# GMichailov/Flash-Attention-CUDA-C

Measured on AMD Instinct MI355X. Metric: fwd attention TFLOP/s/GPU (bf16, seq=4096, d=128) + % MFMA peak, higher is better.
Workload: dtype bf16

## Files before the change

flash-attention-cuda-c_amd/csrc/computers.hip.h:

```cpp
#pragma once

#include "slot_engine.hip.h"

namespace fa {

template <int R>
struct Scores {
    f32x16 s[R][2];
};

template <class C>
struct WaveCompute : SlotEngine<WaveCompute<C>, C> {
    static constexpr int D = C::D, ESZ = C::ESZ, R = 1;
    static constexpr int KS = D / 16;
    static constexpr int DB = D / 32;
    static constexpr int NA = 2 * KS, NB = 4 * DB;
    static constexpr int SA = NA * R, SB = NB * R;
    static constexpr int MPF = ESZ == 1 ? 2 : 1;
    static constexpr int NF = NA / MPF;
    static constexpr int FPH = NF / 2;
    static constexpr int NPRE = C::NPRE < NF ? C::NPRE : NF;
    static constexpr int VPRE = C::VPRE;
    static constexpr int GROUPS = R, RG = 32, LOG_RG = 5, FPG = FPH;
    static constexpr int NE = 32 * R;
    static constexpr int SPAN = SA + (3 * SB) / 4;
    using G = TileGeom<D, ESZ>;
    using Stage = std::conditional_t<C::MIX, MixStage<D, C::NWAVES>,
                  std::conditional_t<C::DMA, DmaStage<D, C::NWAVES, false, true>,
                                     std::conditional_t<C::DMA_K8, HybridStageFp8<D, C::NWAVES>, BufStage<D, ESZ, C::NWAVES, C::PAD>>>>;
    using ScoresT = Scores<R>;
    static constexpr int NL = Stage::NL, NW = Stage::NW;

    u32x4 qf[R][FPH];
    f32x16 o[R][DB];
    float m[R];
    float l[R];
    u32x4 kf[NPRE];
    bf16x8 vf[VPRE + 1];
    uint32_t pw[R][16];
    float sum_a[R], sum_b[R], mx_a[R], mx_b[R], p_even, p_last;
    bool need;
    unsigned long long t_mid = 0, t_end = 0;

    __device__ __forceinline__ void init() {
#pragma unroll
        for (int r = 0; r < R; ++r) {
#pragma unroll
            for (int i = 0; i < DB; ++i)
#pragma unroll
                for (int k = 0; k < 16; ++k) o[r][i][k] = 0.f;
            m[r] = -INFINITY;
            l[r] = 0.f;
        }
    }

    __host__ __device__ static constexpr int frag_u(int f) { return f % FPH; }
    __host__ __device__ static constexpr int frag_kt(int f) { return f / FPH; }
    __device__ __forceinline__ u32x4 k_read(lds_ptr kimg, int kbase, int f) const {
        if constexpr (Stage::K_DMA) return __builtin_bit_cast(u32x4, lds_read_b128(kimg, kbase + frag_kt(f) * (4 * Stage::KBLK) + frag_u(f) * 256));
        else return __builtin_bit_cast(u32x4, lds_read_b128(kimg, kbase + frag_u(f) * 2048 + frag_kt(f) * 512));
    }
    template <int F, int SUB, int RG>
    __device__ __forceinline__ void qk_mfma(const u32x4& kprev, const u32x4& kfrag, Scores<R>& n) const {
        const u32x4& q = qf[RG][frag_u(F)];
        f32x16& acc = n.s[RG][frag_kt(F)];
        if constexpr (C::MXQK) {
            static_assert(ESZ == 1, "the MX form is for fp8 inputs");
            if constexpr ((F & 1) && SUB == MPF - 1) acc = mfma_32x32x64_fp8_unit_scale(kprev, kfrag, qf[RG][(F - 1) % FPH], q, acc);
        } else {
            static_assert(ESZ == 2, "the non-scaled form is for bf16 inputs");
            acc = mfma_32x32x16(__builtin_bit_cast(bf16x8, kfrag), __builtin_bit_cast(bf16x8, q), acc);
        }
    }
    __device__ __forceinline__ static void zero(Scores<R>& n) {
#pragma unroll
        for (int r = 0; r < R; ++r)
#pragma unroll
            for (int k = 0; k < 16; ++k) { n.s[r][0][k] = 0.f; n.s[r][1][k] = 0.f; }
    }

    template <int I = 0>
    __device__ __forceinline__ void qk_all(lds_ptr kimg, int kbase, Scores<R>& n) {
        if constexpr (I == 0) zero(n);
        if constexpr (I < SA) {
            constexpr int f = I / (MPF * R), sub = (I % (MPF * R)) / R, rg = I % R;
            if constexpr (I % (MPF * R) == 0) kf[f % 2] = k_read(kimg, kbase, f);
            qk_mfma<f, sub, rg>(kf[(f + 1) % 2], kf[f % 2], n);
            qk_all<I + 1>(kimg, kbase, n);
        }
    }

    __device__ __forceinline__ void mask(Scores<R>& n, int kv0, int q_row0, int S, int lane) const {
        const int k0 = kv0 + 4 * (lane >> 5);
#pragma unroll
        for (int r = 0; r < R; ++r) {
            const int qi = q_row0 + 32 * r + (lane & 31);
            const int lim = C::CAUSAL ? (qi < S - 1 ? qi : S - 1) : S - 1;
#pragma unroll
            for (int k = 0; k < 16; ++k) {
                n.s[r][0][k] = (k0 + acc_row(k, 0)) > lim ? -INFINITY : n.s[r][0][k];
                n.s[r][1][k] = (k0 + 32 + acc_row(k, 0)) > lim ? -INFINITY : n.s[r][1][k];
            }
        }
    }
    __device__ __forceinline__ float row_max(const Scores<R>& n, int r) const {
        float a = fmaxf(n.s[r][0][0], n.s[r][0][1]), b = fmaxf(n.s[r][1][0], n.s[r][1][1]);
#pragma unroll
        for (int k = 2; k < 16; k += 2) {
            a = fmaxf(a, fmaxf(n.s[r][0][k], n.s[r][0][k + 1]));
            b = fmaxf(b, fmaxf(n.s[r][1][k], n.s[r][1][k + 1]));
        }
        return fmaxf(a, b);
    }
    __device__ __forceinline__ static float max_over_row(float x) { return max_both_halves(x); }

    template <int E, bool F16W = false>
    __device__ __forceinline__ void exp_elem(const Scores<R>& cur, float c) {
        constexpr int g = E / (8 * R), r = (E / 8) % R, j = E % 8, e = 8 * g + j;
        const float x = cur.s[r][e >> 4][e & 15];
        if constexpr (C::LATE_ADD) {
            if constexpr (E > 0) {
                constexpr int rp = ((E - 1) / 8) % R, ep = 8 * ((E - 1) / (8 * R)) + (E - 1) % 8;
                if constexpr (ep & 1) sum_b[rp] += p_last;
                else sum_a[rp] += p_last;
                asm volatile("" : "+v"(sum_a[rp]), "+v"(sum_b[rp]));
            }
            const float p = fast_exp2(fmaf(x, c, -m[r]));
            p_last = p;
            if constexpr (e & 1) pw[r][e >> 1] = F16W ? pack_f16(p_even, p) : pack_bf16(p_even, p);
            else p_even = p;
        } else {
            const float p = fast_exp2(fmaf(x, c, -m[r]));
            if constexpr (e & 1) {
                sum_b[r] += p;
                pw[r][e >> 1] = F16W ? pack_f16(p_even, p) : pack_bf16(p_even, p);
                asm volatile("" : "+v"(sum_a[r]), "+v"(sum_b[r]));
            } else {
                sum_a[r] += p;
                p_even = p;
            }
        }
    }
    __device__ __forceinline__ bf16x8 p_frag(int r, int g) const {
        u32x4 v = {pw[r][4 * g], pw[r][4 * g + 1], pw[r][4 * g + 2], pw[r][4 * g + 3]};
        return __builtin_bit_cast(bf16x8, v);
    }
    template <int J>
    __device__ __forceinline__ void max3_slot(const Scores<R>& n) {
        constexpr int PER = 64 / NB;
#pragma unroll
        for (int k = 0; k < PER; k += 2) {
            const int E = J * PER + k, r = E / 32, e = E % 32;
            const float x0 = n.s[r][e >> 4][e & 15];
            const float x1 = n.s[r][(e + 1) >> 4][(e + 1) & 15];
            if ((k >> 1) & 1) mx_b[r] = fmaxf(fmaxf(mx_b[r], x0), x1);
            else mx_a[r] = fmaxf(fmaxf(mx_a[r], x0), x1);
        }
#pragma unroll
        for (int r = 0; r < R; ++r) asm volatile("" : "+v"(mx_a[r]), "+v"(mx_b[r]));
    }

    __device__ __forceinline__ bf16x8 v_frag(lds_ptr vimg, int vbase, int s4, int db) const {
        const s16x4 lo = lds_read_tr16_b64(vimg, vbase + (2 * s4) * (DB * 512) + db * 512);
        const s16x4 hi = lds_read_tr16_b64(vimg, vbase + (2 * s4 + 1) * (DB * 512) + db * 512);
        typedef __attribute__((ext_vector_type(8))) short s16x8;
        return __builtin_bit_cast(bf16x8, (s16x8)__builtin_shufflevector(lo, hi, 0, 1, 2, 3, 4, 5, 6, 7));
    }

    template <int I, bool F16W = false>
    __device__ __forceinline__ void slots_a(Stage& st, int t_load, lds_ptr k_next, lds_ptr v_cur, int kbase, int vbase,
                                            float c, const Scores<R>& cur, Scores<R>& nxt) {
        if constexpr (I < SA) {
            constexpr int f = I / (MPF * R), rem = I % (MPF * R), sub = rem / R, rg = rem % R;
            if constexpr (C::VALU_FIRST) this->template exp_slot<I, F16W>(cur, c);
            qk_mfma<f, sub, rg>(kf[(f + NPRE - 1) % NPRE], kf[f % NPRE], nxt);
            if constexpr (C::MXQK) {
                if constexpr (rem == MPF * R - 1 && (f & 1)) {
                    if constexpr (f - 1 + NPRE < NF) kf[(f - 1) % NPRE] = k_read(k_next, kbase, f - 1 + NPRE);
                    if constexpr (f + NPRE < NF) kf[f % NPRE] = k_read(k_next, kbase, f + NPRE);
                }
            } else if constexpr (rem == MPF * R - 1 && f + NPRE < NF) {
                kf[f % NPRE] = k_read(k_next, kbase, f + NPRE);
            }
            if constexpr (I >= SA - VPRE) {
                constexpr int v = I - (SA - VPRE);
                vf[v % (VPRE + 1)] = v_frag(v_cur, vbase, v / DB, v % DB);
            }
            this->template load_in_slot<I, F16W>(st, t_load);
            if constexpr (!C::VALU_FIRST) this->template exp_slot<I, F16W>(cur, c);
            __builtin_amdgcn_sched_barrier(0);
            slots_a<I + 1, F16W>(st, t_load, k_next, v_cur, kbase, vbase, c, cur, nxt);
        }
    }
    template <bool TRACK, int J, bool F16W = false>
    __device__ __forceinline__ void slots_b(Stage& st, lds_ptr wr_slot, lds_ptr v_cur, int vbase, float c,
                                            const Scores<R>& cur, const Scores<R>& nxt) {
        if constexpr (J < SB) {
            constexpr int v = J / R, rg = J % R, s4 = v / DB, db = v % DB;
            if constexpr (F16W) o[rg][db] = mfma_32x32x16(__builtin_bit_cast(f16x8, vf[v % (VPRE + 1)]), __builtin_bit_cast(f16x8, p_frag(rg, s4)), o[rg][db]);
            else o[rg][db] = mfma_32x32x16(vf[v % (VPRE + 1)], p_frag(rg, s4), o[rg][db]);
            if constexpr (rg == R - 1 && v + VPRE < NB) {
                constexpr int vn = v + VPRE;
                vf[vn % (VPRE + 1)] = v_frag(v_cur, vbase, vn / DB, vn % DB);
            }
            this->template exp_slot<SA + J, F16W>(cur, c);
            if constexpr (TRACK && J < SB / 2) max3_slot<J>(nxt);
            if constexpr (TRACK && J == SB / 2) this->decide(c);
            this->template write_in_slot<J, F16W>(st, wr_slot);
            __builtin_amdgcn_sched_barrier(0);
            slots_b<TRACK, J + 1, F16W>(st, wr_slot, v_cur, vbase, c, cur, nxt);
        }
    }

    __device__ __forceinline__ void begin_tile(Stage& st, lds_ptr wr_slot, Scores<R>& nxt) {
        st.set_dst(wr_slot);
#pragma unroll
        for (int r = 0; r < R; ++r) {
            sum_a[r] = sum_b[r] = 0.f;
            mx_a[r] = mx_b[r] = -INFINITY;
        }
        zero(nxt);
    }
    __device__ __forceinline__ void end_sums() {
        if constexpr (C::LATE_ADD) {
            static_assert(((NE - 1) % 8) & 1, "the last element feeds sum_b");
            sum_b[((NE - 1) / 8) % R] += p_last;
        }
#pragma unroll
        for (int r = 0; r < R; ++r) l[r] += sum_a[r] + sum_b[r];
    }
    __device__ __forceinline__ void rescale(int r, float alpha) {
        l[r] *= alpha;
#pragma unroll
        for (int i = 0; i < DB; ++i)
#pragma unroll
            for (int k = 0; k < 16; ++k) o[r][i][k] *= alpha;
    }

    __device__ __forceinline__ bool not_finite() const {
        float acc[4] = {0.f, 0.f, 0.f, 0.f};
#pragma unroll
        for (int r = 0; r < R; ++r) {
            acc[0] = fmaf(l[r], 0.f, acc[0]);
#pragma unroll
            for (int i = 0; i < DB; ++i)
#pragma unroll
                for (int k = 0; k < 16; ++k) acc[k & 3] = fmaf(o[r][i][k], 0.f, acc[k & 3]);
        }
        const float a = (acc[0] + acc[1]) + (acc[2] + acc[3]);
        return a != a;
    }

    template <typename OutT>
    __device__ __forceinline__ void store_o_lds(lds_ptr region, char* Oh, float* lse_head, int64_t oS_bytes, int row0, int S,
                                                int lane, int orow_bytes = D * 2) {
        static_assert(sizeof(OutT) == 2, "LDS epilogue is for bf16 / f16 outputs");
        constexpr int ROWB = D * 2, CHUNKS = ROWB / 16;
        const int q = lane & 31, h = lane >> 5;
#pragma unroll
        for (int r = 0; r < R; ++r) {
            const float l_tot = sum_both_halves(l[r]);
            this->store_lse(lse_head, l_tot, r, row0, S, lane);
            const float inv = 1.0f / l_tot;
#pragma unroll
            for (int db = 0; db < DB; ++db)
#pragma unroll
                for (int g4 = 0; g4 < 4; ++g4) {
                    const int d0 = 32 * db + 8 * g4 + 4 * h;
                    const float a = o[r][db][4 * g4 + 0] * inv, b = o[r][db][4 * g4 + 1] * inv;
                    const float c2 = o[r][db][4 * g4 + 2] * inv, e = o[r][db][4 * g4 + 3] * inv;
                    u32x2 v;
                    if constexpr (__is_same(OutT, __bf16)) v = u32x2{pack_bf16(a, b), pack_bf16(c2, e)};
                    else v = u32x2{pack_f16(a, b), pack_f16(c2, e)};
                    const int chunk = (d0 * 2) >> 4, half8 = (d0 * 2) & 8;
                    *reinterpret_cast<FA_LDS u32x2*>(region + (32 * r + q) * ROWB + (((chunk ^ q) & (CHUNKS - 1)) << 4) + half8) = v;
                }
        }
        __builtin_amdgcn_s_waitcnt(0xc07f);
        constexpr int ROWS_PER_INST = 64 / CHUNKS;
        const int rr = lane / CHUNKS, cc = lane % CHUNKS;
        if (!C::PAD && row0 + 32 * R <= S) {
            u32x4 v[32 * R / ROWS_PER_INST];
#pragma unroll
            for (int i = 0; i < 32 * R / ROWS_PER_INST; ++i) {
                const int row = i * ROWS_PER_INST + rr;
                v[i] = *reinterpret_cast<FA_LDS const u32x4*>(region + row * ROWB + (((cc ^ row) & (CHUNKS - 1)) << 4));
            }
#pragma unroll
            for (int i = 0; i < 32 * R / ROWS_PER_INST; ++i)
                store_global_b128<C::O_CACHE>(Oh + (int64_t)(row0 + i * ROWS_PER_INST + rr) * oS_bytes + cc * 16, v[i]);
            return;
        }
#pragma unroll
        for (int i = 0; i < 32 * R / ROWS_PER_INST; ++i) {
            const int row = i * ROWS_PER_INST + rr;
            const u32x4 v = *reinterpret_cast<FA_LDS const u32x4*>(region + row * ROWB + (((cc ^ row) & (CHUNKS - 1)) << 4));
            if (row0 + row < S && (!C::PAD || cc * 16 < orow_bytes))
                *reinterpret_cast<u32x4*>(Oh + (int64_t)(row0 + row) * oS_bytes + cc * 16) = v;
        }
    }
    template <typename OutT>
    __device__ __forceinline__ void store_o_lds32(lds_ptr region, char* Oh, float* lse_head, int64_t oS_bytes, int row0, int S,
                                                  int lane, int orow_bytes = D * 4) {
        static_assert(sizeof(OutT) == 4, "for fp32 outputs");
        const int q = lane & 31, h = lane >> 5;
        float inv[R];
#pragma unroll
        for (int r = 0; r < R; ++r) {
            const float l_tot = sum_both_halves(l[r]);
            this->store_lse(lse_head, l_tot, r, row0, S, lane);
            inv[r] = 1.0f / l_tot;
        }
        const int rr = lane >> 4, cc = lane & 15;
#pragma unroll
        for (int hf = 0; hf < D / 64; ++hf) {
            if (hf > 0) __builtin_amdgcn_s_waitcnt(0xc07f);
#pragma unroll
            for (int r = 0; r < R; ++r)
#pragma unroll
                for (int dd = 0; dd < 2; ++dd)
#pragma unroll
                    for (int g4 = 0; g4 < 4; ++g4) {
                        const int db = 2 * hf + dd, cidx = 8 * dd + 2 * g4 + h;
                        const f32x4 v = {o[r][db][4 * g4 + 0] * inv[r], o[r][db][4 * g4 + 1] * inv[r],
                                         o[r][db][4 * g4 + 2] * inv[r], o[r][db][4 * g4 + 3] * inv[r]};
                        *reinterpret_cast<FA_LDS f32x4*>(region + (32 * r + q) * 256 + (((cidx ^ q) & 15) << 4)) = v;
                    }
            __builtin_amdgcn_s_waitcnt(0xc07f);
            if (!C::PAD && row0 + 32 * R <= S) {
                f32x4 v[8 * R];
#pragma unroll
                for (int i = 0; i < 8 * R; ++i) v[i] = *reinterpret_cast<FA_LDS const f32x4*>(region + (4 * i + rr) * 256 + (((cc ^ (4 * i + rr)) & 15) << 4));
#pragma unroll
                for (int i = 0; i < 8 * R; ++i) store_global_b128<C::O_CACHE>(Oh + (int64_t)(row0 + 4 * i + rr) * oS_bytes + hf * 256 + cc * 16, __builtin_bit_cast(u32x4, v[i]));
                continue;
            }
#pragma unroll
            for (int i = 0; i < 8 * R; ++i) {
                const int row = 4 * i + rr;
                const f32x4 v = *reinterpret_cast<FA_LDS const f32x4*>(region + row * 256 + (((cc ^ row) & 15) << 4));
                if (row0 + row < S && (!C::PAD || hf * 256 + cc * 16 < orow_bytes))
                    *reinterpret_cast<f32x4*>(Oh + (int64_t)(row0 + row) * oS_bytes + hf * 256 + cc * 16) = v;
            }
        }
    }
};

}
```

flash-attention-cuda-c_amd/csrc/kernel_bf16.hip.h:

```cpp
#pragma once

#include "computers.hip.h"
#include "computers16.hip.h"

#include <type_traits>

namespace fa {

struct Opt {
    bool stamp = false;
    bool pad = false;
    int m16 = -1;
    int sum_mfma = -1;
    int waves = 8;
    bool p_f16 = false;
    bool mix = false;
    int kv_clamp = -1;
    int q_nt = -1;
};

template <int D_, bool CAUSAL_, typename OutT_, int ESZ_ = 2, Opt O = Opt{}>
struct KernelCfg {
    static constexpr int D = D_;
    static constexpr bool CAUSAL = CAUSAL_;
    using OutT = OutT_;
    static constexpr int ESZ = ESZ_;
    static constexpr bool STAMP = O.stamp, PAD = O.pad;
    static constexpr bool PRIO_A = true;
    static constexpr int O_CACHE = CAUSAL_ ? 2 : 0;
    static constexpr int Q_CACHE = (O.q_nt < 0 ? CAUSAL_ : O.q_nt != 0) ? 2 : 0;
    static constexpr bool KV_CLAMP = CAUSAL_ && O.kv_clamp != 0;
    static constexpr bool COALESCED_Q = D_ == 128 && !O.pad;
    static constexpr bool MXQK = ESZ_ == 1;
    static constexpr bool M16 = (O.m16 < 0 ? true : O.m16 != 0) && ESZ_ == 2;
    static constexpr bool SUM_MFMA = M16 && (O.sum_mfma < 0 ? true : O.sum_mfma != 0);
    static constexpr bool VALU_FIRST = !M16;
    static constexpr bool P_F16 = M16 && O.p_f16;
    static constexpr bool LATE_ADD = !M16;
    static constexpr bool DMA = ESZ_ == 2 && !O.pad && !O.p_f16;
    static constexpr bool MIX = O.mix && DMA;
    static_assert(!O.mix || (ESZ_ == 2 && !O.pad && !O.p_f16 && (O.m16 == 0 || O.sum_mfma == 0)),
                  "the mixed-precision kernels are the LDS-DMA kernels (16x16x32 engine: with fp32 row sums)");
    static constexpr bool DMA_K8 = ESZ_ == 1 && D_ == 128 && !O.pad && O.waves == 8;
    static constexpr int NPRE = 4;
    static constexpr int VPRE = 2;
    static constexpr int THR = 8;
    static constexpr int NWAVES = O.waves;
    static_assert(NWAVES == 8 || NWAVES == 4, "8 or 4 waves");
    static constexpr int QBLK = 32 * NWAVES;
    static constexpr int RING = 3;
    static constexpr int RING_BYTES = RING * TileGeom<D_, ESZ_>::SLOT;
    static constexpr int EP_OFF = (DMA || DMA_K8) ? TileGeom<D_, ESZ_>::SLOT : 0;
    static constexpr int EP_NEED = EP_OFF + (sizeof(OutT_) == 2 ? QBLK * D_ * 2 : QBLK * 256);
    static constexpr int FLAG_OFF = EP_NEED > RING_BYTES ? EP_NEED : RING_BYTES;
    static constexpr int LDS_BYTES = FLAG_OFF + 64;
    static_assert(LDS_BYTES <= 163840, "160 KiB of LDS per CU");
};

template <int D, bool CAUSAL, typename OutT, int ESZ = 2, bool STAMP = false, bool PAD = false, bool LSE = false>
using ProdCfg = KernelCfg<D, CAUSAL, OutT, ESZ, Opt{.stamp = STAMP, .pad = PAD, .m16 = CAUSAL ? 0 : -1, .sum_mfma = LSE ? 0 : -1}>;

template <int NWAVES>
__device__ __forceinline__ bool block_or(bool v, lds_ptr flags, int wave) {
    const uint32_t mine = __any(v) ? 1u : 0u;
    *reinterpret_cast<FA_LDS uint32_t*>(flags + 4 * wave) = mine;
    __syncthreads();
    u32x4 a = *reinterpret_cast<FA_LDS const u32x4*>(flags);
    uint32_t r = a[0] | a[1] | a[2] | a[3];
    if constexpr (NWAVES == 8) {
        const u32x4 b = *reinterpret_cast<FA_LDS const u32x4*>(flags + 16);
        r |= b[0] | b[1] | b[2] | b[3];
    }
    return __builtin_amdgcn_readfirstlane(r) != 0;
}

template <int D, typename OutT, bool STAMP = false>
using MixCfg = KernelCfg<D, true, OutT, 2, Opt{.stamp = STAMP, .m16 = 0, .mix = true}>;

template <class C>
using WaveComputeOf = std::conditional_t<C::M16, WaveCompute16<C>, WaveCompute<C>>;

template <class C, bool TRACK, bool F16W = C::P_F16>
__device__ __forceinline__ bool attention_pass(const Params& p, WaveComputeOf<C>& w, typename WaveComputeOf<C>::Stage& st, lds_ptr smem,
                                               int n_tiles, int my_tiles, int q_row0, int lane,
                                               unsigned long long (&acc)[24], bool tile0_in_flight) {
    using G = TileGeom<C::D, C::ESZ>;
    constexpr bool CAUSAL = C::CAUSAL;
    constexpr int KVBLK = 64, SLOT = G::SLOT, KT = G::K_TILE;
    const int S = p.Sk;
    unsigned long long tp0 = 0, tp1 = 0, tp2 = 0;
    if constexpr (C::STAMP) tp0 = cycle_stamp();
    w.init();
    using WC = WaveComputeOf<C>;
    constexpr int KBLK = (G::ROWB / 16) * 128;
    const int kbase = WC::Stage::K_DMA ? (C::M16 ? kd16_read_base(lane, KBLK) : kd_read_base(lane, KBLK)) : (C::M16 ? k16_read_base(lane) : k_read_base(lane));
    const int vbase = C::M16 ? v16_read_base<C::D>(lane) : v_read_base(lane);
    const float c = p.scale_log2;
    auto needs_mask = [&](int t) { return (CAUSAL && t * KVBLK + KVBLK - 1 > q_row0) || (t * KVBLK + KVBLK > S); };
    typename WC::ScoresT sA, sB;

    if (!tile0_in_flight) st.template load_all_into<F16W>(0, smem);
    st.template write_all<F16W>(smem);
    unsigned long long tw0 = 0;
    if constexpr (C::STAMP) tw0 = cycle_stamp();
    st.wait_all();
    if constexpr (C::STAMP) acc[16] += cycle_stamp() - tw0;
    __syncthreads();
    st.template load_all_into<F16W>(1, smem + SLOT);
    constexpr int AHEAD = C::RING - 1;
    if constexpr (C::STAMP) tp1 = cycle_stamp();
    if (my_tiles > 0) {
        w.qk_all(smem, kbase, sA);
        if (needs_mask(0)) w.mask(sA, 0, q_row0, S, lane);
        w.first_max(sA, c);
    }
    st.template write_all<F16W>(smem + SLOT);
    st.wait_all();
    __syncthreads();
    if constexpr (C::STAMP) { tp2 = cycle_stamp(); acc[8] += tp1 - tp0; acc[9] += tp2 - tp1; }

    int so_cur = 0, so_nxt = SLOT, so_wr = AHEAD * SLOT;
    auto step = [&](int t, int kind, typename WC::ScoresT& cur, typename WC::ScoresT& nxt) {
        unsigned long long t0 = 0, t4 = 0, t6 = 0;
        if constexpr (C::STAMP) t0 = cycle_stamp();
        if (kind != 2) {
            const bool has_next = kind == 0;
            w.template tile_step<TRACK, F16W>(st, t + AHEAD, smem + so_wr, smem + so_nxt, smem + so_cur + KT, kbase, vbase, c, cur, nxt,
                                              has_next, has_next && needs_mask(t + 1), (t + 1) * KVBLK, q_row0, S, lane);
        } else {
            st.template load_all_into<F16W>(t + AHEAD, smem + so_wr);
            st.template write_all<F16W>(smem + so_wr);
        }
        if constexpr (C::STAMP) t4 = cycle_stamp();
        st.wait_all();
        __syncthreads();
        if constexpr (C::STAMP) {
            t6 = cycle_stamp();
            if (kind != 2) { acc[1] += w.t_mid - t0; acc[2] += w.t_end - w.t_mid; acc[3] += t4 - w.t_end; acc[6] += 1; }
            acc[5] += t6 - t4;
        }
        const int tmp = so_cur;
        so_cur = so_nxt;
        so_nxt = so_wr;
        so_wr = tmp;
    };
    auto kind_of = [&](int t) { return t + 1 < my_tiles ? 0 : (t < my_tiles ? 1 : 2); };
    for (int t = 0; t < n_tiles; t += 2) {
        step(t, kind_of(t), sA, sB);
        if (t + 1 < n_tiles) step(t + 1, kind_of(t + 1), sB, sA);
    }
    if constexpr (TRACK && !F16W) return false;
    else {
        unsigned long long tc0 = 0;
        if constexpr (C::STAMP) tc0 = cycle_stamp();
        const bool bad = block_or<C::NWAVES>(my_tiles > 0 && w.not_finite(), smem + C::FLAG_OFF, __builtin_amdgcn_readfirstlane(threadIdx.x >> 6));
        if constexpr (C::STAMP) acc[10] += cycle_stamp() - tc0;
        return bad;
    }
}

template <class C>
__device__ __forceinline__ bool work_unit(const UnitList& p, int round, int& g, int& qb) {
    const int bid = blockIdx.x;
    int idx = bid >> 3;
    idx = round * p.jpx + ((round & 1) ? p.jpx - 1 - idx : idx);
    if (idx >= p.cpx) return false;
    const int u = (bid & 7) * p.cpx + idx;
    if (u >= p.units) return false;
    g = u / p.nQ;
    qb = u - g * p.nQ;
    if (C::CAUSAL) qb = p.nQ - 1 - qb;
    qb += p.qb0;
    return true;
}

template <class C>
struct UnitCtx {
    const char *Qh, *Kh, *Vh;
    char* Oh;
    float* lse_head;
    int q_row0, n_tiles, my_tiles;
    bool wave_live;
    bool early;
    __device__ __forceinline__ void set(const Params& p, int g, int qb, int wave) {
        early = C::MIX && qb < p.hp;
        constexpr int ESZ = C::ESZ, KVBLK = 64, QBLK = C::QBLK, WROWS = 32;
        const int b = g / p.H, h = g - b * p.H, hk = kv_head(p, h);
        Qh = (const char*)p.Q + (b * p.qB + h * p.qH) * ESZ;
        Kh = (const char*)p.K + (b * p.kB + hk * p.kH) * ESZ;
        Vh = (const char*)p.V + (b * p.vB + hk * p.vH) * ESZ;
        Oh = (char*)p.O + (b * p.oB + h * p.oH) * (int64_t)sizeof(typename C::OutT);
        lse_head = p.lse ? p.lse + (int64_t)g * p.S : nullptr;
        q_row0 = qb * QBLK + wave * WROWS;
        const int q_end = min(p.S, (qb + 1) * QBLK);
        const int k_tiles = (p.Sk + KVBLK - 1) / KVBLK;
        n_tiles = C::CAUSAL ? min(k_tiles, (q_end + KVBLK - 1) / KVBLK) : k_tiles;
        wave_live = q_row0 < p.S;
        my_tiles = !wave_live ? 0 : (C::CAUSAL ? min(n_tiles, (q_row0 + WROWS - 1) / KVBLK + 1) : n_tiles);
    }
    __device__ __forceinline__ int kv_rows(int Sk) const { return C::KV_CLAMP ? min(Sk, 64 * n_tiles) : Sk; }
};

template <class C, bool F16W>
__device__ __forceinline__ void run_passes(const Params& p, WaveComputeOf<C>& w, typename WaveComputeOf<C>::Stage& st, lds_ptr smem,
                                           const UnitCtx<C>& u, int lane, unsigned long long (&acc)[24]) {
    if (!attention_pass<C, false, F16W>(p, w, st, smem, u.n_tiles, u.my_tiles, u.q_row0, lane, acc, true)) return;
    if constexpr (F16W) {
        if (!attention_pass<C, true, true>(p, w, st, smem, u.n_tiles, u.my_tiles, u.q_row0, lane, acc, false)) return;
    }
    attention_pass<C, true, false>(p, w, st, smem, u.n_tiles, u.my_tiles, u.q_row0, lane, acc, false);
}

enum class Kind { ALL, ONE };
template <class C, Kind KIND>
__device__ __forceinline__ bool next_unit(const UnitList& L, int& round, int& g, int& qb) {
    if constexpr (KIND == Kind::ALL) return work_unit<C>(L, round, g, qb);
    else {
        g = L.units;
        qb = L.qb0;
        return round == 0;
    }
}

template <class C, Kind KIND = Kind::ALL>
__device__ __forceinline__ void run_units(const Params& p, const UnitList& L, lds_ptr smem) {
    constexpr int D = C::D, ESZ = C::ESZ;
    using OutT = typename C::OutT;

    int g, qb, round = 0;
    if (!next_unit<C, KIND>(L, round, g, qb)) return;
    unsigned long long t_kernel0 = 0, t_real0 = 0;
    if constexpr (C::STAMP) { t_real0 = realtime_stamp(); t_kernel0 = cycle_stamp(); }
    const int lane = threadIdx.x & 63;
    const int wave = __builtin_amdgcn_readfirstlane(threadIdx.x >> 6);
    const int S = p.S, Sk = p.Sk;
    const int64_t qSb = p.qS * ESZ, kSb = p.kS * ESZ, vSb = p.vS * ESZ, oSb = p.oS * (int64_t)sizeof(OutT);
    constexpr int WROWS = 32;

    UnitCtx<C> cur;
    cur.set(p, g, qb, wave);
    WaveComputeOf<C> w;
    typename WaveComputeOf<C>::Stage st;
    const int row_bytes = C::PAD ? p.d * ESZ : D * ESZ, orow_bytes = C::PAD ? p.d * (int)sizeof(OutT) : D * (int)sizeof(OutT);
    st.init(cur.Kh, cur.Vh, kSb, vSb, cur.kv_rows(Sk), wave, lane, row_bytes);
    if (C::MIX ? cur.early : C::P_F16) st.template load_all_into<true>(0, smem);
    else st.template load_all_into<false>(0, smem);
    if constexpr (C::COALESCED_Q) w.load_q_rows(cur.Qh, qSb, cur.q_row0, S, lane);
    else w.load_q(cur.Qh, qSb, cur.q_row0, S, lane, row_bytes);
    unsigned long long acc[24] = {0, 0, 0, 0, 0, 0, 0, 0, 0, 0, 0, 0, 0, 0, 0, 0, 0, 0, 0, 0, 0, 0, 0, 0};
    if constexpr (C::STAMP) acc[12] = cycle_stamp() - t_kernel0;

    while (true) {
        unsigned long long t_q0 = 0;
        if constexpr (C::STAMP) t_q0 = cycle_stamp();
        w.pin_q();
        if constexpr (C::COALESCED_Q) {
            using G = TileGeom<D, ESZ>;
            static_assert(G::SLOT + C::QBLK * D * ESZ <= C::LDS_BYTES, "Q staging regions must fit behind slot 0");
            int lane_q = lane;
            asm volatile("" : "+v"(lane_q));
            w.q_rows_to_fragments(smem + G::SLOT + wave * (WROWS * D * ESZ), lane_q);
            w.pin_q();
        }
        if constexpr (C::STAMP) acc[7] += cycle_stamp() - t_q0;

        int lane_p = lane;
        asm volatile("" : "+v"(lane_p));
        if (C::MIX ? cur.early : C::P_F16) {
            if constexpr (C::MIX || C::P_F16) run_passes<C, true>(p, w, st, smem, cur, lane_p, acc);
        } else {
            run_passes<C, false>(p, w, st, smem, cur, lane_p, acc);
        }

        unsigned long long t_nx0 = 0;
        if constexpr (C::STAMP) t_nx0 = cycle_stamp();
        UnitCtx<C> nxt;
        ++round;
        const bool more = next_unit<C, KIND>(L, round, g, qb);
        if (more) {
            nxt.set(p, g, qb, wave);
            st.init(nxt.Kh, nxt.Vh, kSb, vSb, nxt.kv_rows(Sk), wave, lane, row_bytes);
            if (C::MIX ? nxt.early : C::P_F16) st.template load_all_into<true>(0, smem);
            else st.template load_all_into<false>(0, smem);
            int lane_n = lane;
            asm volatile("" : "+v"(lane_n));
            if constexpr (C::COALESCED_Q) w.load_q_rows(nxt.Qh, qSb, nxt.q_row0, S, lane_n);
            else w.load_q(nxt.Qh, qSb, nxt.q_row0, S, lane_n, row_bytes);
            __builtin_amdgcn_sched_barrier(0);
        }

        unsigned long long t_ep0 = 0;
        if constexpr (C::STAMP) { t_ep0 = cycle_stamp(); acc[13] += t_ep0 - t_nx0; }
        int lane_e = lane;
        asm volatile("" : "+v"(lane_e));
        if constexpr (sizeof(OutT) == 2) {
            static_assert(C::EP_OFF + C::QBLK * D * 2 <= C::LDS_BYTES, "epilogue regions must fit the ring");
            if (cur.wave_live)
                w.template store_o_lds<OutT>(smem + C::EP_OFF + wave * (WROWS * D * 2), cur.Oh, cur.lse_head, oSb, cur.q_row0, S, lane_e, orow_bytes);
        } else {
            static_assert(C::EP_OFF + C::QBLK * 64 * 4 <= C::LDS_BYTES, "epilogue regions must fit the ring");
            if (cur.wave_live)
                w.template store_o_lds32<OutT>(smem + C::EP_OFF + wave * (WROWS * 256), cur.Oh, cur.lse_head, oSb, cur.q_row0, S, lane_e, orow_bytes);
        }
        if constexpr (C::STAMP) acc[4] += cycle_stamp() - t_ep0;
        if (!more) break;
        unsigned long long t_b0 = 0;
        if constexpr (C::STAMP) t_b0 = cycle_stamp();
        if constexpr (!C::DMA) __syncthreads();
        if constexpr (C::STAMP) acc[15] += cycle_stamp() - t_b0;
        cur = nxt;
    }
    if constexpr (C::STAMP) {
        const unsigned long long t_tail0 = cycle_stamp();
        asm volatile("s_waitcnt vmcnt(0)" ::: "memory");
        const unsigned long long t_end = cycle_stamp();
        acc[14] = t_end - t_tail0;
        acc[0] = t_end - t_kernel0;
        const unsigned long long t_real1 = realtime_stamp();
        acc[17] = t_real1 - t_real0;
        acc[18] = t_real0;
        acc[19] = t_real1;
        if (lane == 0 && p.dbg) {
            acc[11] = 1;
#pragma unroll
            for (int k = 0; k < 24; ++k) p.dbg[((size_t)blockIdx.x * 8 + wave) * 24 + k] = acc[k];
        }
    }
}

template <class C>
__global__ __launch_bounds__(64 * C::NWAVES, 2) void fwd_mfma_kernel(const Params p) {
    extern __shared__ __attribute__((aligned(16))) char smem_raw[];
    run_units<C>(p, unit_list_of(p), (lds_ptr)smem_raw);
}

template <class CA, class CB>
__global__ __launch_bounds__(64 * CA::NWAVES, (CA::LDS_BYTES > 81920 || CB::LDS_BYTES > 81920) ? 1 : 2) void fwd_mfma_pair_kernel(const Params p, const int hp, const int jpx) {
    static_assert(CA::NWAVES == 4 && CB::NWAVES == 4 && CA::CAUSAL == CB::CAUSAL, "one workgroup shape, one mask");
    extern __shared__ __attribute__((aligned(16))) char smem_raw[];
    const int x = blockIdx.x & 7, s = blockIdx.x >> 3;
    const int heads = p.B * p.H, hpx = (heads + 7) / 8;
    const int h0 = x * hpx, nh = min(hpx, heads - h0);
    if (nh <= 0) return;
    const int n = nh * p.nQ;
    const int idx = s < jpx ? s : n - 1 - (s - jpx);
    if (idx >= n || (s >= jpx && idx < jpx)) return;
    const int blk = idx / nh;
    const UnitList one{p.nQ, p.nQ - 1 - blk, h0 + (idx - blk * nh), 0, 0};
    if constexpr (std::is_same_v<CA, CB>) {
        run_units<CA, Kind::ONE>(p, one, (lds_ptr)smem_raw);
    } else {
        if (one.qb0 < hp) run_units<CB, Kind::ONE>(p, one, (lds_ptr)smem_raw);
        else run_units<CA, Kind::ONE>(p, one, (lds_ptr)smem_raw);
    }
}

}
```

flash-attention-cuda-c_amd/csrc/slot_engine.hip.h:

```cpp
#pragma once

#include "loaders.hip.h"

namespace fa {

template <class W, class C>
struct SlotEngine {
    __device__ __forceinline__ W& self() { return *static_cast<W*>(this); }

    __host__ __device__ static constexpr int elem_slot(int E) { return E * W::SPAN / W::NE; }
    __host__ __device__ static constexpr int load_slot(int n) { return 1 + 2 * n; }
    __host__ __device__ static constexpr int wstep() { return 2 * W::NW <= W::SB / 2 + 1 ? 2 : 1; }
    template <int SLOT, bool F16W = false, int N = 0, class St>
    __device__ __forceinline__ void load_in_slot(St& st, int t_load) {
        if constexpr (N < W::NL) {
            if constexpr (load_slot(N) == SLOT) st.template load<N, F16W>(t_load);
            load_in_slot<SLOT, F16W, N + 1>(st, t_load);
        }
    }
    template <int J, bool F16W = false, class St>
    __device__ __forceinline__ void write_in_slot(St& st, lds_ptr wr_slot) {
        constexpr int H = W::SB / 2, WSTEP = wstep();
        static_assert(2 * W::NL <= W::SA && WSTEP * (W::NW - 1) < W::SB - H, "staging does not fit the slot plan");
        if constexpr (J >= H && (J - H) % WSTEP == 0 && (J - H) / WSTEP < W::NW) st.template write<(J - H) / WSTEP, F16W>(wr_slot);
    }
    template <int SLOT, bool F16W = false, int E = 0, class Sc>
    __device__ __forceinline__ void exp_slot(const Sc& cur, float c) {
        if constexpr (E < W::NE) {
            if constexpr (elem_slot(E) == SLOT) self().template exp_elem<E, F16W>(cur, c);
            exp_slot<SLOT, F16W, E + 1>(cur, c);
        }
    }

    __device__ __forceinline__ void load_q(const char* Qh, int64_t qS_bytes, int row0, int S, int lane, int row_bytes = C::D * C::ESZ) {
        W& w = self();
        constexpr int FSTRIDE = (64 / W::RG) * 16;
#pragma unroll
        for (int g = 0; g < W::GROUPS; ++g) {
            int row = row0 + W::RG * g + (lane & (W::RG - 1));
            row = row < S ? row : S - 1;
            const char* src = Qh + row * qS_bytes + (lane >> W::LOG_RG) * 16;
#pragma unroll
            for (int u = 0; u < W::FPG; ++u) {
                if constexpr (C::PAD) {
                    w.qf[g][u] = u32x4{0u, 0u, 0u, 0u};
                    if (u * FSTRIDE + (lane >> W::LOG_RG) * 16 < row_bytes) w.qf[g][u] = load_global_b128<C::Q_CACHE>(src + u * FSTRIDE);
                } else {
                    w.qf[g][u] = load_global_b128<C::Q_CACHE>(src + u * FSTRIDE);
                }
            }
        }
    }
    static constexpr int QCH = (C::D * C::ESZ) / 16, QRPI = 64 / QCH;
    __device__ __forceinline__ void load_q_rows(const char* Qh, int64_t qS_bytes, int row0, int S, int lane) {
        static_assert(32 / QRPI == W::GROUPS * W::FPG, "coalesced Q: as many loads as fragments");
#pragma unroll
        for (int i = 0; i < W::GROUPS * W::FPG; ++i) {
            int row = row0 + i * QRPI + lane / QCH;
            row = row < S ? row : S - 1;
            self().qf[i / W::FPG][i % W::FPG] = load_global_b128<C::Q_CACHE>(Qh + row * qS_bytes + (lane % QCH) * 16);
        }
    }
    __device__ __forceinline__ void q_rows_to_fragments(lds_ptr region, int lane) {
        W& w = self();
        constexpr int ROWB = C::D * C::ESZ;
#pragma unroll
        for (int i = 0; i < W::GROUPS * W::FPG; ++i) {
            const int q = i * QRPI + lane / QCH, c = lane % QCH;
            lds_write_b128(region, q * ROWB + (((c ^ q) & (QCH - 1)) << 4), w.qf[i / W::FPG][i % W::FPG]);
        }
        asm volatile("s_waitcnt lgkmcnt(0)" ::: "memory");
#pragma unroll
        for (int g = 0; g < W::GROUPS; ++g)
#pragma unroll
            for (int u = 0; u < W::FPG; ++u) {
                const int q = W::RG * g + (lane & (W::RG - 1)), c = (64 / W::RG) * u + (lane >> W::LOG_RG);
                w.qf[g][u] = __builtin_bit_cast(u32x4, lds_read_b128(region, q * ROWB + (((c ^ q) & (QCH - 1)) << 4)));
            }
    }
    __device__ __forceinline__ void pin_q() {
#pragma unroll
        for (int g = 0; g < W::GROUPS; ++g)
#pragma unroll
            for (int u = 0; u < W::FPG; ++u) asm volatile("" : "+v"(self().qf[g][u]));
    }

    template <class Sc>
    __device__ __forceinline__ void first_max(const Sc& n, float c) {
        W& w = self();
#pragma unroll
        for (int g = 0; g < W::GROUPS; ++g) w.m[g] = fmaxf(w.m[g], W::max_over_row(w.row_max(n, g)) * c);
    }
    __device__ __forceinline__ void decide(float c) {
        W& w = self();
        bool any = false;
#pragma unroll
        for (int g = 0; g < W::GROUPS; ++g) {
            const float mx = W::max_over_row(fmaxf(w.mx_a[g], w.mx_b[g])) * c;
            any = any || (mx > w.m[g] + (float)C::THR);
            w.mx_a[g] = mx;
        }
        w.need = __any(any);
    }

    template <bool TRACK, bool F16W = false, class St, class Sc>
    __device__ __forceinline__ void tile_step(St& st, int t_load, lds_ptr wr_slot, lds_ptr k_next, lds_ptr v_cur, int kbase, int vbase, float c,
                                              const Sc& cur, Sc& nxt, bool has_next, bool mask_next, int kv0_next, int q_row0, int S, int lane) {
        W& w = self();
        w.begin_tile(st, wr_slot, nxt);
#pragma unroll
        for (int i = 0; i < W::NPRE; ++i) w.kf[i] = w.k_read(k_next, kbase, i);
        if constexpr (C::PRIO_A) __builtin_amdgcn_s_setprio(1);
        __builtin_amdgcn_sched_barrier(0);
        w.template slots_a<0, F16W>(st, t_load, k_next, v_cur, kbase, vbase, c, cur, nxt);
        if constexpr (C::PRIO_A) {
            __builtin_amdgcn_s_setprio(0);
            __builtin_amdgcn_sched_barrier(0);
        }
        if constexpr (C::STAMP) w.t_mid = cycle_stamp();
        w.template slots_b<TRACK, 0, F16W>(st, wr_slot, v_cur, vbase, c, cur, nxt);
        if constexpr (C::STAMP) w.t_end = cycle_stamp();
        w.end_sums();
        if (has_next && mask_next) {
            w.mask(nxt, kv0_next, q_row0, S, lane);
            if constexpr (TRACK) {
#pragma unroll
                for (int g = 0; g < W::GROUPS; ++g) { w.mx_a[g] = w.row_max(nxt, g); w.mx_b[g] = w.mx_a[g]; }
                decide(c);
            }
        }
        if constexpr (TRACK) {
            if (has_next && w.need) {
#pragma unroll
                for (int g = 0; g < W::GROUPS; ++g) {
                    const float mn = fmaxf(w.m[g], w.mx_a[g]);
                    const float alpha = fast_exp2(w.m[g] - mn);
                    w.m[g] = mn;
                    w.rescale(g, alpha);
                }
            }
        }
    }

    __device__ __forceinline__ void store_lse(float* lse_head, float l_tot, int g, int row0, int S, int lane) {
        const int qi = row0 + W::RG * g + (lane & (W::RG - 1));
        if (lse_head && lane < W::RG && qi < S) lse_head[qi] = (self().m[g] + __builtin_amdgcn_logf(l_tot)) * 0.6931471805599453f;
    }
};

}
```

Measured before the change: 1078.

## Add specialized last-tile tail step for causal mixed kernels with half-tile skip

Adds a dedicated tail_step for the last KV tile of each query block. It skips the next-tile QK and row-max tracking and front-loads the V fragment, load and exp work into a lead-in. With TAIL_HALF it also skips the upper half of the PV MFMAs when the diagonal tile is half masked. The default only enables this for causal kernels using the mix option with m16=0, so the fwd bf16 path in this metric may not use it. It adds code size and a branch on the half condition.

```diff
diff --git a/flash-attention-cuda-c_amd/csrc/computers.hip.h b/flash-attention-cuda-c_amd/csrc/computers.hip.h
--- a/flash-attention-cuda-c_amd/csrc/computers.hip.h
+++ b/flash-attention-cuda-c_amd/csrc/computers.hip.h
@@ -212,6 +212,45 @@
         }
     }
 
+    __host__ __device__ static constexpr int tail_elem_slot(int E) { return (E / 8 - 1) * DB + (E % 8) * DB / 8; }
+    template <int E, bool F16W = false>
+    __device__ __forceinline__ void tail_pre(Stage& st, int t_load, lds_ptr v_cur, int vbase, float c, const Scores<R>& cur) {
+        static_assert(R == 1 && NL <= 8 && VPRE <= DB, "tail step: one row group, the lead-in carries every piece");
+        if constexpr (E < 8) {
+            if constexpr (E < VPRE) vf[E % (VPRE + 1)] = v_frag(v_cur, vbase, E / DB, E % DB);
+            if constexpr (E < NL) st.template load<E, F16W>(t_load);
+            this->template exp_elem<E, F16W>(cur, c);
+            tail_pre<E + 1, F16W>(st, t_load, v_cur, vbase, c, cur);
+        }
+    }
+    template <int J, int ST, int E = 8, bool F16W = false>
+    __device__ __forceinline__ void tail_exp(const Scores<R>& cur, float c) {
+        if constexpr (E < 8 * (ST / DB)) {
+            if constexpr (tail_elem_slot(E) == J) this->template exp_elem<E, F16W>(cur, c);
+            tail_exp<J, ST, E + 1, F16W>(cur, c);
+        }
+    }
+    template <int J, int J1, int ST, bool F16W = false>
+    __device__ __forceinline__ void slots_t(lds_ptr v_cur, int vbase, float c, const Scores<R>& cur) {
+        if constexpr (J < J1) {
+            constexpr int s4 = J / DB, db = J % DB;
+            if constexpr (F16W) o[0][db] = mfma_32x32x16(__builtin_bit_cast(f16x8, vf[J % (VPRE + 1)]), __builtin_bit_cast(f16x8, p_frag(0, s4)), o[0][db]);
+            else o[0][db] = mfma_32x32x16(vf[J % (VPRE + 1)], p_frag(0, s4), o[0][db]);
+            if constexpr (J + VPRE < ST) {
+                constexpr int vn = J + VPRE;
+                vf[vn % (VPRE + 1)] = v_frag(v_cur, vbase, vn / DB, vn % DB);
+            }
+            tail_exp<J, ST, 8, F16W>(cur, c);
+            __builtin_amdgcn_sched_barrier(0);
+            slots_t<J + 1, J1, ST, F16W>(v_cur, vbase, c, cur);
+        }
+    }
+    __device__ __forceinline__ void begin_tail(Stage& st, lds_ptr wr_slot) {
+        st.set_dst(wr_slot);
+#pragma unroll
+        for (int r = 0; r < R; ++r) sum_a[r] = sum_b[r] = 0.f;
+    }
+
     __device__ __forceinline__ void begin_tile(Stage& st, lds_ptr wr_slot, Scores<R>& nxt) {
         st.set_dst(wr_slot);
 #pragma unroll
diff --git a/flash-attention-cuda-c_amd/csrc/kernel_bf16.hip.h b/flash-attention-cuda-c_amd/csrc/kernel_bf16.hip.h
--- a/flash-attention-cuda-c_amd/csrc/kernel_bf16.hip.h
+++ b/flash-attention-cuda-c_amd/csrc/kernel_bf16.hip.h
@@ -17,6 +17,8 @@
     bool mix = false;
     int kv_clamp = -1;
     int q_nt = -1;
+    int tail = -1;
+    int tail_half = -1;
 };
 
 template <int D_, bool CAUSAL_, typename OutT_, int ESZ_ = 2, Opt O = Opt{}>
@@ -30,6 +32,8 @@
     static constexpr int O_CACHE = CAUSAL_ ? 2 : 0;
     static constexpr int Q_CACHE = (O.q_nt < 0 ? CAUSAL_ : O.q_nt != 0) ? 2 : 0;
     static constexpr bool KV_CLAMP = CAUSAL_ && O.kv_clamp != 0;
+    static constexpr bool TAIL = ESZ_ == 2 && O.m16 == 0 && (O.tail < 0 ? CAUSAL_ && O.mix : O.tail != 0);
+    static constexpr bool TAIL_HALF = TAIL && CAUSAL_ && O.tail_half != 0;
     static constexpr bool COALESCED_Q = D_ == 128 && !O.pad;
     static constexpr bool MXQK = ESZ_ == 1;
     static constexpr bool M16 = (O.m16 < 0 ? true : O.m16 != 0) && ESZ_ == 2;
@@ -120,10 +124,13 @@
     if constexpr (C::STAMP) { tp2 = cycle_stamp(); acc[8] += tp1 - tp0; acc[9] += tp2 - tp1; }
 
     int so_cur = 0, so_nxt = SLOT, so_wr = AHEAD * SLOT;
-    auto step = [&](int t, int kind, typename WC::ScoresT& cur, typename WC::ScoresT& nxt) {
+    auto step = [&]<bool TAIL_SITE = false>(int t, int kind, typename WC::ScoresT& cur, typename WC::ScoresT& nxt) {
         unsigned long long t0 = 0, t4 = 0, t6 = 0;
         if constexpr (C::STAMP) t0 = cycle_stamp();
-        if (kind != 2) {
+        if constexpr (TAIL_SITE) {
+            const bool half = C::TAIL_HALF && (q_row0 & 63) == 0 && t * KVBLK + 32 > q_row0 + 31;
+            w.template tail_step<F16W>(st, t + AHEAD, smem + so_wr, smem + so_cur + KT, vbase, c, cur, half);
+        } else if (kind != 2) {
             const bool has_next = kind == 0;
             w.template tile_step<TRACK, F16W>(st, t + AHEAD, smem + so_wr, smem + so_nxt, smem + so_cur + KT, kbase, vbase, c, cur, nxt,
                                               has_next, has_next && needs_mask(t + 1), (t + 1) * KVBLK, q_row0, S, lane);
@@ -145,9 +152,26 @@
         so_wr = tmp;
     };
     auto kind_of = [&](int t) { return t + 1 < my_tiles ? 0 : (t < my_tiles ? 1 : 2); };
-    for (int t = 0; t < n_tiles; t += 2) {
-        step(t, kind_of(t), sA, sB);
-        if (t + 1 < n_tiles) step(t + 1, kind_of(t + 1), sB, sA);
+    if constexpr (C::TAIL && !TRACK) {
+        const int last = my_tiles - 1;
+        for (int t = 0; t < last; t += 2) {
+            step(t, 0, sA, sB);
+            if (t + 1 < last) step(t + 1, 0, sB, sA);
+        }
+        if (last >= 0) {
+            if (last & 1) sA = sB;
+            step.template operator()<true>(last, 1, sA, sB);
+        }
+        for (int t = my_tiles; t < n_tiles; ++t) {
+            int ts = t;
+            asm volatile("" : "+s"(ts));
+            step(ts, 2, sA, sB);
+        }
+    } else {
+        for (int t = 0; t < n_tiles; t += 2) {
+            step(t, kind_of(t), sA, sB);
+            if (t + 1 < n_tiles) step(t + 1, kind_of(t + 1), sB, sA);
+        }
     }
     if constexpr (TRACK && !F16W) return false;
     else {
diff --git a/flash-attention-cuda-c_amd/csrc/slot_engine.hip.h b/flash-attention-cuda-c_amd/csrc/slot_engine.hip.h
--- a/flash-attention-cuda-c_amd/csrc/slot_engine.hip.h
+++ b/flash-attention-cuda-c_amd/csrc/slot_engine.hip.h
@@ -142,6 +142,28 @@
         }
     }
 
+    template <bool HALF, bool F16W, class Sc>
+    __device__ __forceinline__ void tail_rest(lds_ptr v_cur, int vbase, float c, const Sc& cur) {
+        constexpr int DB = W::DB, ST = (HALF ? 2 : 4) * DB;
+        self().template slots_t<DB, ST, ST, F16W>(v_cur, vbase, c, cur);
+    }
+    template <bool F16W = false, class St, class Sc>
+    __device__ __forceinline__ void tail_step(St& st, int t_load, lds_ptr wr_slot, lds_ptr v_cur, int vbase, float c, const Sc& cur, bool half) {
+        W& w = self();
+        constexpr int DB = W::DB;
+        w.begin_tail(st, wr_slot);
+        __builtin_amdgcn_sched_barrier(0);
+        w.template tail_pre<0, F16W>(st, t_load, v_cur, vbase, c, cur);
+        __builtin_amdgcn_sched_barrier(0);
+        if constexpr (C::STAMP) w.t_mid = cycle_stamp();
+        w.template slots_t<0, DB, 2 * DB, F16W>(v_cur, vbase, c, cur);
+        if (half) tail_rest<true, F16W>(v_cur, vbase, c, cur);
+        else tail_rest<false, F16W>(v_cur, vbase, c, cur);
+        st.template write_all<F16W>(wr_slot);
+        if constexpr (C::STAMP) w.t_end = cycle_stamp();
+        w.end_sums();
+    }
+
     __device__ __forceinline__ void store_lse(float* lse_head, float l_tot, int g, int row0, int S, int lane) {
         const int qi = row0 + W::RG * g + (lane & (W::RG - 1));
         if (lse_head && lane < W::RG && qi < S) lse_head[qi] = (self().m[g] + __builtin_amdgcn_logf(l_tot)) * 0.6931471805599453f;
```

Measured after the change: 1092, median of 6. +1.3%, better.
